# jacarvalho/mpd-public

Measured on AMD Instinct MI355X. Metric: denoising-steps/s, higher is better.
Workload: dtype f32; 1 GPU; cfg2: EnvDense2D-RobotPointMass shape, 100 trajectories (1 context(s)) x H=64 x D=4, T=100 (+5) reverse steps, unguided, U-Net dim_mults (1, 2, 4, 8), one plan = one bench step; parallelism=single, denoising_steps_per_plan=105

## Files before the change

### include/mpdx.h

```cpp
#ifndef MPDX_H
#define MPDX_H

#include <stddef.h>
#include <stdint.h>

#ifdef __cplusplus
extern "C" {
#endif

#define MPDX_E_INVALID   (-1)
#define MPDX_E_NOTFOUND  (-2)
#define MPDX_E_STATE     (-3)
#define MPDX_E_DEVICE    (-4)

#define MPDX_MAX_LEVELS 8

typedef struct mpdx_unet mpdx_unet;

typedef struct mpdx_unet_cfg {
    int32_t state_dim;
    int32_t n_support_points;
    int32_t unet_input_dim;
    int32_t n_levels;
    int32_t dim_mults[MPDX_MAX_LEVELS];
    int32_t time_emb_dim;
    int32_t self_attention;
} mpdx_unet_cfg;

const char* mpdx_last_error(void);
int mpdx_version(void);

int    mpdx_unet_create(const mpdx_unet_cfg* cfg, mpdx_unet** out);
void   mpdx_unet_destroy(mpdx_unet* u);
int    mpdx_unet_set_plan_join(mpdx_unet* u, int on);
int    mpdx_unet_plan_joined(const mpdx_unet* u);
int    mpdx_unet_set_inner_run(mpdx_unet* u, int on);
int    mpdx_unet_set_inner_run_parts(mpdx_unet* u, int parts);
int    mpdx_unet_inner_runs(const mpdx_unet* u);
int    mpdx_unet_inner_run_layers(const mpdx_unet* u);
int    mpdx_unet_status(const mpdx_unet* u);
int    mpdx_unet_set_status(mpdx_unet* u, unsigned word);
int    mpdx_unet_num_params(const mpdx_unet* u);
int    mpdx_unet_param_info(const mpdx_unet* u, int idx, const char** name, int32_t shape[3], int32_t* ndim);
size_t mpdx_unet_packed_floats(const mpdx_unet* u);
size_t mpdx_unet_timetab_floats(const mpdx_unet* u, int T);
size_t mpdx_unet_workspace_floats(const mpdx_unet* u, int B);
int    mpdx_unet_pack_param(mpdx_unet* u, const char* name, const float* src_dev, size_t n_floats,
                            float* packed_dev, void* stream);
int    mpdx_unet_build_timetab(mpdx_unet* u, const float* packed_dev, const float* freqs16_dev, int T,
                               float* timetab_dev, void* stream);

int mpdx_unet_forward(mpdx_unet* u, const float* packed_dev, const float* timetab_dev, int T,
                      const float* x, int t, float* eps, int B, float* ws, void* stream);

typedef struct mpdx_step_coefs {
    float sqrt_recip_alphas_cumprod;
    float sqrt_recipm1_alphas_cumprod;
    float posterior_mean_coef1;
    float posterior_mean_coef2;
    float noise_scale;
// ... 214 lines not shown
```

### mpd_public_amd/_lib.py

```python
from __future__ import annotations

import ctypes as C
from pathlib import Path

import os as _os

_LIB_PATH = Path(_os.environ["MPDX_LIB"]) if _os.environ.get("MPDX_LIB") else Path(__file__).resolve().parent / "libmpdx.so"
_lib = None

MAX_LEVELS = 8


class UnetCfg(C.Structure):
    _fields_ = [("state_dim", C.c_int32), ("n_support_points", C.c_int32), ("unet_input_dim", C.c_int32),
                ("n_levels", C.c_int32), ("dim_mults", C.c_int32 * MAX_LEVELS), ("time_emb_dim", C.c_int32),
                ("self_attention", C.c_int32)]


class StepCoefs(C.Structure):
    _fields_ = [("sqrt_recip_alphas_cumprod", C.c_float), ("sqrt_recipm1_alphas_cumprod", C.c_float),
                ("posterior_mean_coef1", C.c_float), ("posterior_mean_coef2", C.c_float),
                ("noise_scale", C.c_float), ("noise_std_extra", C.c_float),
                ("predict_epsilon", C.c_int32), ("clip_denoised", C.c_int32), ("ddim_k1", C.c_float), ("ddim_k2", C.c_float),
                ("guide_scale", C.c_float)]
# ... 38 lines not shown


class RrtOpts(C.Structure):
    _fields_ = [("q_lo", C.c_float * 8), ("q_hi", C.c_float * 8), ("step", C.c_float), ("max_nodes", C.c_int32), ("max_iters", C.c_int32),
                ("max_connect_steps", C.c_int32), ("n_edge_checks", C.c_int32), ("seed", C.c_uint64)]


class IkOpts(C.Structure):
    _fields_ = [("frame", C.c_int32), ("offset", C.c_float * 3), ("q_lo", C.c_float * 8), ("q_hi", C.c_float * 8), ("rot_weight", C.c_float),
                ("pos_tol", C.c_float), ("rot_tol", C.c_float), ("lambda_init", C.c_float), ("lambda_up", C.c_float), ("lambda_down", C.c_float),
                ("lambda_min", C.c_float), ("lambda_max", C.c_float), ("adaptive", C.c_int32), ("max_iters", C.c_int32), ("seed", C.c_uint64)]


_vp, _sz, _i, _f = C.c_void_p, C.c_size_t, C.c_int, C.c_float
SIGNATURES = {
    "mpdx_last_error": (C.c_char_p, []),
    "mpdx_version": (_i, []),
    "mpdx_unet_create": (_i, [C.POINTER(UnetCfg), C.POINTER(_vp)]),
    "mpdx_unet_destroy": (None, [_vp]),
    "mpdx_unet_set_plan_join": (_i, [_vp, _i]),
    "mpdx_unet_plan_joined": (_i, [_vp]),
    "mpdx_unet_set_inner_run": (_i, [_vp, _i]),
    "mpdx_unet_set_inner_run_parts": (_i, [_vp, _i]),
    "mpdx_unet_inner_runs": (_i, [_vp]),
    "mpdx_unet_inner_run_layers": (_i, [_vp]),
    "mpdx_unet_status": (_i, [_vp]),
    "mpdx_unet_set_status": (_i, [_vp, C.c_uint]),
    "mpdx_unet_num_params": (_i, [_vp]),
    "mpdx_unet_param_info": (_i, [_vp, _i, C.POINTER(C.c_char_p), C.POINTER(C.c_int32 * 3), C.POINTER(C.c_int32)]),
    "mpdx_unet_packed_floats": (_sz, [_vp]),
    "mpdx_unet_timetab_floats": (_sz, [_vp, _i]),
    "mpdx_unet_workspace_floats": (_sz, [_vp, _i]),
    "mpdx_unet_pack_param": (_i, [_vp, C.c_char_p, _vp, _sz, _vp, _vp]),
    "mpdx_unet_build_timetab": (_i, [_vp, _vp, _vp, _i, _vp, _vp]),
    "mpdx_unet_forward": (_i, [_vp, _vp, _vp, _i, _vp, _i, _vp, _i, _vp, _vp]),
    "mpdx_ddpm_step": (_i, [_vp, _vp, _vp, _i, _vp, _vp, _vp, _vp, C.POINTER(StepCoefs), _i, _i, _vp, _vp, _i, _i, _vp, _vp]),
    "mpdx_add_noise": (_i, [_vp, _vp, _vp, _vp, _f, _f, _vp, _i, _i, _i, _vp]),
    "mpdx_hard_conds": (_i, [_vp, _vp, _i, C.POINTER(C.c_int32), C.POINTER(_vp), _i, _i, _i, _vp]),
    "mpdx_q_sample": (_i, [_vp, _vp, _vp, _vp, _vp, _vp, _vp, _vp, _i, _i, _i, _i, _vp]),
    "mpdx_weighted_loss": (_i, [_vp, _vp, _vp, _vp, _vp, _i, _vp, _i, _i, _i, _vp]),
    "mpdx_plan": (_i, [_vp, _vp, _vp, _i, C.POINTER(StepCoefs), _i, _vp, _vp, _vp, _vp, _vp, _i, _vp,
                        C.POINTER(GuideParams), _i, _i, _vp, _i, C.c_uint64, C.c_uint64, _vp]),
    "mpdx_guide_step": (_i, [C.POINTER(GuideParams), _vp, _vp, _vp, _vp, _vp, _vp, _i, _i, _i, _i, _vp]),
    "mpdx_guide_step_scaled": (_i, [C.POINTER(GuideParams), _vp, _vp, _vp, _vp, _vp, _vp, _i, _i, _i, _i, _f, _vp]),
    "mpdx_guide_time": (_i, [C.POINTER(GuideParams), _vp, _vp, _vp, _i, _i, _i, _i, _i, _vp, C.POINTER(C.c_float)]),
    "mpdx_traj_metrics": (_i, [C.POINTER(GuideParams), _vp, _vp, _i, _i, _i, _i, _vp]),
# ... 85 lines not shown
```

### mpd_public_amd/csrc/host.hpp

```cpp
#pragma once
#include <hip/hip_runtime.h>

#include <algorithm>
#include <cmath>
#include <cstdarg>
#include <cstdio>
#include <cstdlib>
#include <cstring>
#include <mutex>
#include <set>
#include <string>
#include <unordered_map>
#include <vector>

#include "../../include/mpdx.h"
#include "conv_block.hpp"
#include "conv_ws.hpp"
#include "fused_level.hpp"
#include "switches.hpp"
#include "train_types.hpp"

namespace mpdx {

int fail(int code, const char* fmt, ...);
// ... 55 lines not shown
    bool pin_nt = false;
    std::string name;
};

}

struct mpdx_unet {
    mpdx_unet_cfg cfg;
    std::vector<mpdx::Param> params;
    std::unordered_map<std::string, int> pidx;
    std::vector<mpdx::Layer> layers;
    size_t packed_floats = 0;
    size_t slot_floats = 0;
    int n_slots = 0;
    int tt_row = 0;
    std::vector<int> tt_w, tt_b, tt_cout, tt_off;
    int final_slot = 0;
    int n_done = 0;
    int Hc = 0, xpad_slot = -1;
    bool masked() const { return Hc != cfg.n_support_points; }
    int plan_join = 1;
    enum RunPart { kRunSeven = 1, kRunTail = 2 };
    int inner_run = kRunSeven | kRunTail;
    int plan_joined = 0, inner_runs = 0;
    int inner_run_layers = 0;
    struct InnerRunState {
        int capacity = -1;
        bool seven_ok = false, tail_ok = false;
        long long budget = 0;
        unsigned* counters = nullptr;
        unsigned base = 0;
        int live = 1 << 30;
        bool rezero = false;
        unsigned *status = nullptr, *status_dev = nullptr;
        unsigned status_host = 0;
        unsigned status_word() const { return status ? __atomic_load_n(status, __ATOMIC_RELAXED) : status_host; }
    } run;
    struct CopyJob { size_t src, dst; int n0, ss0, ds0, n1, ss1, ds1, n_inner; };
    struct Fused {
        int first = 0, count = 0;
        bool has_final = false;
        int in1 = 0, in2 = 0;
        int in3 = mpdx::SRC_NONE;
        int gout_slot[3] = {-1, -1, -1};
        size_t lds_bytes = 0;
        mpdx::FusedArgs tmpl;
        int program = -1;
        std::vector<CopyJob> jobs;
        std::vector<int> op_layer;
        int in3_consumer = -1;
    };
    std::vector<Fused> fused;
    void* jobs_dev = nullptr;
    int n_jobs = 0;
    const float* streams_for = nullptr;
    int pack_version = 0, streams_version = -1;
    enum UnitKind { kProgram, kLayer, kPair, kInnerRun, kTailRun };
    struct Unit { UnitKind kind; int fused; int layer; int count; };
    std::vector<int> owner;
    struct TrainLayer {
        int src1_l = -2, src2_l = -2, res_l = -2;
        bool need_dgrad = false;
        size_t dgrad_woff = 0;
        mpdx::Layer dg;
    };
    bool train_ready = false;
    size_t flat_floats = 0, packedT_floats = 0;
    std::vector<TrainLayer> tl;
    std::vector<mpdx::PackDesc> pack_descs_host;
    void* pack_descs_dev = nullptr;
    void* pack_chunks_dev = nullptr;
    size_t n_pack_chunks = 0;
};

namespace mpdx {

int pick_row_stride(int cin_pad, int mode, int L_in, int L_out, int LP);
void choose_tile(const Layer& l, int B, int& MT, int& NT);
bool layer_ksplit(const Layer& l);
int check_ready(const mpdx_unet* u);
unsigned fused_mask(int B);
bool fused_save_variant(const mpdx_unet::Fused& f);
int ensure_fused_streams(mpdx_unet* u, const float* packed, hipStream_t st);
int claim_fused_stream_jobs(mpdx_unet* u, const float* packed, const void** jobs, int* n);
int launch_final_step(const FinalArgs& fa, hipStream_t st);
int launch_conv_layer(const Layer& l, ConvArgs& a, int B, hipStream_t st);
bool pair_tile(const Layer& l1, const Layer& l2, int B, int& MT, int& NT);
int launch_conv_pair(int MT, int NT, const ConvArgs& a1, const ConvArgs& a2, const Layer& l1, const Layer& l2, hipStream_t st);
template <int N> struct RunArgs;
int inner_run_grid(int B);
int inner_run_workgroups_per_cu();
int tail_run_workgroups_per_cu();
int launch_inner_run(const RunArgs<7>& ra, int B, hipStream_t st);
int launch_tail_run(const RunArgs<4>& ra, int B, hipStream_t st);
struct AttnArgs;
const char* attn_unsupported(int C, int L);
int launch_attention(const Layer& l, AttnArgs& a, int B, hipStream_t st);
int launch_weight_stationary(int variant, const Layer& l, ConvArgs& a, const ConvArgs& a2, int B, hipStream_t st);
int launch_fused_args(const mpdx_unet::Fused& f, const FusedArgs& a, int B, hipStream_t st, bool save = false);
int launch_fused_train(const mpdx_unet::Fused& f, const FusedArgs& a, int B, hipStream_t st);
int launch_fused_join(const FusedJoinArgs& ja, int B, hipStream_t st);
size_t fused_join_lds_bytes();
struct NoiseRng;
int launch_guide(const mpdx_guide_params* gp, float* x, float* grad_out, const float* hs, const float* hg, const uint32_t* amax_in,
                 uint32_t* amax_out, int n_per_ctx, int B, int H, int D, hipStream_t st, const float* noise = nullptr, float noise_scale = 0.f,
                 float noise_extra = 0.f, float* chain = nullptr, float guide_scale = 1.0f, const NoiseRng* rng = nullptr);
const char* chain_params_problem(const mpdx_guide_params& gp);
const char* tool_params_problem(const mpdx_guide_params& gp);
struct ChainInfo;
int guide_block_problem(const mpdx_guide_params* gp, int D, ChainInfo* chain_info);

}
```

### mpd_public_amd/csrc/inner_run.hpp

```cpp
#pragma once
#include "conv_block.hpp"

namespace mpdx {

constexpr int kInnerRunLayers = 7;
constexpr int kTailRunLayers = 4;
constexpr int kInnerRunCounterStride = 32;

template <int N>
struct RunArgs {
    ConvArgs layer[N];
    unsigned* counters;
    unsigned* status;
    long long budget;
    unsigned base;
    int n_layers;
    int nc;
};
typedef RunArgs<kInnerRunLayers> InnerRunArgs;
typedef RunArgs<kTailRunLayers> TailRunArgs;

constexpr size_t run_max(size_t a, size_t b) { return a > b ? a : b; }

struct RunSeqSeven {
    typedef InnerRunArgs Args;
    static constexpr int kLayers = kInnerRunLayers;
    static constexpr bool kUp = false;
    static constexpr int kLastL = 8, kLastMT = 32, kLastC = 256;
    static __device__ __forceinline__ bool gn(const ConvArgs& a, int id, const RunCtx& rc) { return conv_block_body<CONV_S1, 5, EPI_GN_MISH, 32, 32, 1, 8, GeoL8<16>, -1, true>(a, id, rc); }
    static __device__ __forceinline__ bool up(const ConvArgs&, int, const RunCtx&) { return true; }
    static __device__ __forceinline__ int tiled(int) { return 0; }
    static size_t lds() { return conv_block_lds_bytes<CONV_S1, 5, 32, 32, 8>(8, 8, 256 + 8) + 16; }
};
struct RunSeqTail {
    typedef TailRunArgs Args;
    static constexpr int kLayers = kTailRunLayers;
    static constexpr bool kUp = true;
    static constexpr int kLastL = 16, kLastMT = 16, kLastC = 128;
    static __device__ __forceinline__ bool gn(const ConvArgs& a, int id, const RunCtx& rc) { return conv_block_body<CONV_S1, 5, EPI_GN_MISH, 16, 32, 1, 8, GeoL8<8>, -1, true>(a, id, rc); }
    static __device__ __forceinline__ bool up(const ConvArgs& a, int id, const RunCtx& rc) { return conv_block_body<CONV_UPT, 4, EPI_BIAS, 16, 64, 1, 8, GeoUp8<8>, -1, true>(a, id, rc); }
    static __device__ __forceinline__ int tiled(int i) { return i >= 3 ? 1 : ((i > 0 ? 1 : 0) | (i == 2 ? 2 : 0) | 4); }
    static size_t lds() { return run_max(conv_block_lds_bytes<CONV_S1, 5, 16, 32, 8>(8, 8, 128 + 8), conv_block_lds_bytes<CONV_UPT, 4, 16, 64, 8>(8, 16, 128 + 4)) + 16; }
};

template <class SEQ>
__device__ __forceinline__ void run_give_up(const typename SEQ::Args& ra, const RunCtx& rc, const int c, const int m, const int i) {
    const int tid = threadIdx.x;
    if (tid == 0) {
        __hip_atomic_fetch_or(ra.status, 1u | ((unsigned)i << 8), __ATOMIC_RELAXED, __HIP_MEMORY_SCOPE_SYSTEM);
        __hip_atomic_store(rc.counter, rc.target + kRunPoison, __ATOMIC_RELAXED, __HIP_MEMORY_SCOPE_AGENT);
    }
    const ConvArgs& last = ra.layer[ra.n_layers - 1];
    constexpr int L = SEQ::kLastL, MT = SEQ::kLastMT;
    for (int e = tid; e < 4 * L * MT; e += 512) {
        const int b = c * 4 + (e >> geo_ilog2(L * MT)), l = (e >> geo_ilog2(MT)) & (L - 1), ch = m * MT + (e & (MT - 1));
        if (b < last.B) last.dst[((size_t)b * L + l) * SEQ::kLastC + ch] = __builtin_nanf("");
    }
}

template <class SEQ, bool SAME_XCD>
__global__ __launch_bounds__(512) void inner_run_kernel(const typename SEQ::Args ra) {
    int c, m;
    if constexpr (SAME_XCD) {
        const int b = blockIdx.x, x = b & 7, r = b >> 3;
        m = r & 7; c = (r >> 3) * 8 + x;
        if (c >= ra.nc) return;
    } else {
        c = (int)blockIdx.x >> 3; m = blockIdx.x & 7;
    }
    warm_kernarg<sizeof(typename SEQ::Args)>();
    RunCtx rc;
    rc.counter = ra.counters + (size_t)c * kInnerRunCounterStride;
    rc.budget = ra.budget;
    const int n_gn = SEQ::kUp ? ra.n_layers - 1 : ra.n_layers;
#pragma nounroll
    for (int i = 0; i < n_gn; ++i) {
        rc.wait = i > 0;
        rc.target = ra.base + 8u * (unsigned)i;
        rc.tiled = SEQ::tiled(i);
        if (SEQ::gn(ra.layer[i], c * 8 + m, rc)) continue;
        run_give_up<SEQ>(ra, rc, c, m, i);
        return;
    }
    if constexpr (SEQ::kUp) {
        rc.wait = n_gn > 0;
        rc.target = ra.base + 8u * (unsigned)n_gn;
        rc.tiled = SEQ::tiled(n_gn);
        if (!SEQ::up(ra.layer[n_gn], c * 8 + m, rc)) run_give_up<SEQ>(ra, rc, c, m, n_gn);
    }
}

// ... 2 lines not shown
```

### mpd_public_amd/csrc/k_inner_run.hip

```cpp
#include "host.hpp"
#include "inner_run.hpp"

namespace mpdx {

#ifndef MPDX_INNER_RUN_SAME_XCD
#define MPDX_INNER_RUN_SAME_XCD 1
#endif
static constexpr bool kSameXcd = MPDX_INNER_RUN_SAME_XCD != 0;

int inner_run_grid(int B) {
    const int nc = (B + 3) / 4;
    return kSameXcd ? ((nc + 7) / 8) * 64 : nc * 8;
}

template <class SEQ>
static int workgroups_per_cu() {
    int n = 0;
    if (hipOccupancyMaxActiveBlocksPerMultiprocessor(&n, (const void*)inner_run_kernel<SEQ, kSameXcd>, 512, SEQ::lds()) != hipSuccess) {
        (void)hipGetLastError();
        return 0;
    }
    return n;
}
int inner_run_workgroups_per_cu() { return workgroups_per_cu<RunSeqSeven>(); }
int tail_run_workgroups_per_cu() { return workgroups_per_cu<RunSeqTail>(); }

template <class SEQ>
static int launch_run(const typename SEQ::Args& ra, int B, hipStream_t st, const char* what) {
    if (ra.n_layers != SEQ::kLayers || ra.nc != (B + 3) / 4) return fail(MPDX_E_INVALID, "%s: %d layers, %d clusters for B=%d", what, ra.n_layers, ra.nc, B);
    hipLaunchKernelGGL((inner_run_kernel<SEQ, kSameXcd>), dim3(inner_run_grid(B)), dim3(512), SEQ::lds(), st, ra);
    return 0;
}
int launch_inner_run(const InnerRunArgs& ra, int B, hipStream_t st) { return launch_run<RunSeqSeven>(ra, B, st, "inner run"); }
int launch_tail_run(const TailRunArgs& ra, int B, hipStream_t st) { return launch_run<RunSeqTail>(ra, B, st, "tail run"); }

}
```

### mpd_public_amd/csrc/mpdx.hip

```cpp
#include "host.hpp"
#include "attn.hpp"
#include "inner_run.hpp"
#include "loss.hpp"
#include "scene_table.hpp"

namespace mpdx {

static thread_local char g_err[512] = "";
int fail(int code, const char* fmt, ...) {
    va_list ap;
    va_start(ap, fmt);
    vsnprintf(g_err, sizeof(g_err), fmt, ap);
    va_end(ap);
    return code;
}

int raise_lds_limit(const void* kern) {
    static std::mutex mu;
    static std::set<std::pair<int, const void*>> done;
    int dev = 0;
    HIP_TRY(hipGetDevice(&dev));
    std::lock_guard<std::mutex> lock(mu);
    if (done.count({dev, kern})) return 0;
    HIP_TRY(hipFuncSetAttribute(kern, hipFuncAttributeMaxDynamicSharedMemorySize, 160 * 1024));
// ... 676 lines not shown
}
static int run_fused(mpdx_unet* u, const mpdx_unet::Fused& f, const float* packed, const float* tt_row, const float* x, float* ws,
                     int B, const FinalArgs* fa, hipStream_t st) {
    if (int rc = ensure_fused_streams(u, packed, st)) return rc;
    FusedArgs a;
    if (int rc = fill_fused_args(u, f, packed, tt_row, x, ws, B, fa, a)) return rc;
    return launch_fused_args(f, a, B, st);
}
static int run_fused_join(mpdx_unet* u, const mpdx_unet::Fused& up, const mpdx_unet::Fused& dn, const float* packed, const float* tt_row, const float* tt_next,
                          const float* x, float* ws, int B, const FinalArgs* fa, hipStream_t st, long long* trace = nullptr) {
    if (int rc = ensure_fused_streams(u, packed, st)) return rc;
    FusedJoinArgs ja;
    FusedArgs d;
    if (int rc = fill_fused_args(u, up, packed, tt_row, x, ws, B, fa, ja.up)) return rc;
    if (int rc = fill_fused_args(u, dn, packed, tt_next, x, ws, B, nullptr, d)) return rc;
    ja.up.trace = trace;
    ja.dn.packed = d.packed; ja.dn.tt_row = d.tt_row;
    for (int k = 0; k < 3; ++k) ja.dn.gout[k] = d.gout[k];
    ja.dn.gpar_off = d.gpar_off; ja.dn.tt_lo = d.tt_lo;
    for (int k = 0; k < kMaxFusedOps; ++k) ja.dn.sbase[k] = k < d.nops ? d.ops[k].sbase : 0;
    return launch_fused_join(ja, B, st);
}

static size_t inner_run_counter_bytes(int capacity) { return (size_t)((capacity + 7) / 8 + 8) * kInnerRunCounterStride * sizeof(unsigned); }
static int inner_run_create(mpdx_unet::InnerRunState& r, int cus) {
    if (r.capacity >= 0) return 0;
    r.capacity = 0;
    int dev = 0, khz = 0;
    if (cus <= 0 || hipGetDevice(&dev) != hipSuccess || hipDeviceGetAttribute(&khz, hipDeviceAttributeClockRate, dev) != hipSuccess)
        return (void)hipGetLastError(), 0;
    r.seven_ok = inner_run_workgroups_per_cu() > 0;
    r.tail_ok = tail_run_workgroups_per_cu() > 0;
    if (!r.seven_ok && !r.tail_ok) return 0;
    HIP_TRY(hipMalloc((void**)&r.counters, inner_run_counter_bytes(cus)));
    HIP_TRY(hipMemset(r.counters, 0, inner_run_counter_bytes(cus)));
    HIP_TRY(hipHostMalloc((void**)&r.status, 64, hipHostMallocMapped));
    *r.status = r.status_host;
    HIP_TRY(hipHostGetDevicePointer((void**)&r.status_dev, r.status, 0));
    r.budget = 4LL * (khz > 0 ? khz : 2400000);
    r.capacity = cus;
    return 0;
}
static int inner_run_begin(mpdx_unet::InnerRunState& r, int nc, int n_layers, hipStream_t st, unsigned* base_out) {
    if (r.rezero || nc > r.live) {
        HIP_TRY(hipMemsetAsync(r.counters, 0, inner_run_counter_bytes(r.capacity), st));
        r.base = 0; r.rezero = false;
    }
    r.live = nc;
    *base_out = r.base;
    r.base += 8u * (unsigned)n_layers;
    return 0;
}
static void inner_run_free(mpdx_unet::InnerRunState& r) {
    if (r.counters) (void)hipFree(r.counters);
    if (r.status) (void)hipHostFree(r.status);
}
static int handle_status_error(const mpdx_unet* u, const char* fn) {
    const unsigned w = u->run.status_word();
    if (!w) return 0;
    return fail(MPDX_E_DEVICE, "%s: a workgroup of the inner-level run gave up its wait (status 0x%x: layer %u of the run); the outputs of that plan hold NaN. "
                "mpdx_unet_set_status(u, 0) clears the word", fn, w, w >> 8);
}
static long long* g_run_trace = nullptr;
static int g_run_trace_kind = -1;
constexpr int kRunTraceSlots = 32;
template <int N>
static int fill_run_args(mpdx_unet* u, int kind, int first, const float* packed, const float* row, const float* x, float* ws, int B, hipStream_t st, RunArgs<N>& ra) {
    memset(&ra, 0, sizeof(ra));
    for (int k = 0; k < N; ++k) {
        if (int rc = make_conv_args(u, u->layers[first + k], packed, row, x, ws, B, 0, ra.layer[k])) return rc;
        ra.layer[k].n_tiles_n = (B + 3) / 4;
        ra.layer[k].trace = g_run_trace && g_run_trace_kind == kind ? g_run_trace + k * kRunTraceSlots : nullptr;
    }
    ra.n_layers = N; ra.nc = (B + 3) / 4;
    if (int rc = inner_run_begin(u->run, ra.nc, N, st, &ra.base)) return rc;
    ra.counters = u->run.counters; ra.status = u->run.status_dev; ra.budget = u->run.budget;
    u->inner_run_layers += N;
    return 0;
}
static int run_inner_run(mpdx_unet* u, int first, const float* packed, const float* row, const float* x, float* ws, int B, hipStream_t st) {
    InnerRunArgs ra;
    if (int rc = fill_run_args(u, mpdx_unet::kInnerRun, first, packed, row, x, ws, B, st, ra)) return rc;
    u->inner_runs++;
    return launch_inner_run(ra, B, st);
}
static int run_tail_run(mpdx_unet* u, int first, int spare, const float* packed, const float* row, const float* x, float* ws, int B, hipStream_t st) {
    TailRunArgs ra;
    if (spare < 0 || spare >= u->n_slots) return fail(MPDX_E_STATE, "tail run without a spare slot");
    if (int rc = fill_run_args(u, mpdx_unet::kTailRun, first, packed, row, x, ws, B, st, ra)) return rc;
    float* const sp = ws + u->slot_floats * (size_t)B * spare;
    ra.layer[0].dst = sp; ra.layer[1].src1 = sp; ra.layer[2].res = sp;
    return launch_tail_run(ra, B, st);
}

static int run_unit(mpdx_unet* u, const mpdx_unet::Unit& un, const float* packed, const float* row, const float* x, float* ws, int B,
                    const FinalArgs* fa, hipStream_t st) {
    if (un.kind == mpdx_unet::kProgram) return run_fused(u, u->fused[un.fused], packed, row, x, ws, B, fa, st);
    if (un.kind == mpdx_unet::kPair) return run_pair(u, u->layers[un.layer], u->layers[un.layer + 1], packed, row, x, ws, B, st);
    if (un.kind == mpdx_unet::kInnerRun) return run_inner_run(u, un.layer, packed, row, x, ws, B, st);
    if (un.kind == mpdx_unet::kTailRun) return run_tail_run(u, un.layer, un.fused, packed, row, x, ws, B, st);
    return run_layer(u, u->layers[un.layer], packed, row, x, ws, B, st);
}
static double unit_flops(const mpdx_unet* u, const mpdx_unet::Unit& un, int B) {
    double fl = 0.0;
    for (int k = un.layer; k < un.layer + un.count; ++k) fl += layer_flops(u->layers[k], B);
    return fl;
}

static double layer_param_bytes(const mpdx_unet* u, const Layer& l) {
    if (l.attn) return 4.0 * ((double)u->params[l.w].n + (double)u->params[l.w2].n + 3.0 * l.cout);
    double n = (double)u->params[l.w].n + l.cout;
    if (l.gamma >= 0) n += 2.0 * l.cout;
    if (l.tb_off >= 0) n += l.cout;
    return 4.0 * n;
}
static double unit_bytes(const mpdx_unet* u, const mpdx_unet::Unit& un, int B) {
    auto act = [&](int L, int C) { return 4.0 * B * (double)L * C; };
    if (un.kind == mpdx_unet::kProgram) {
        const auto& f = u->fused[un.fused];
        const Layer& l0 = u->layers[f.first];
        double b = act(l0.L_in, l0.c1 + l0.c2);
        if (f.in3_consumer >= 0) b += act(u->layers[f.in3_consumer].L_in, u->layers[f.in3_consumer].c2);
        for (int k = f.first; k < f.first + f.count; ++k) b += layer_param_bytes(u, u->layers[k]);
// ... 111 lines not shown
        }
        if (read_later || held(u->final_slot)) continue;
        auto named = [&](const Layer& l, int s) { return l.src1 == s || l.src2 == s || l.res == s || l.dst == s; };
        for (int s = 0; s < u->n_slots && *spare < 0; ++s) {
            if (s == u->xpad_slot || named(l0, s) || named(l1, s) || named(l2, s) || named(l3, s)) continue;
            bool dead = s != u->final_slot;
            for (int j = f + kTailRunLayers; j < (int)u->layers.size() && dead; ++j) {
                const Layer& l = u->layers[j];
                if (l.src1 == s || l.src2 == s || l.res == s) dead = false;
                else if (l.dst == s) break;
            }
            if (dead) *spare = s;
        }
        if (*spare < 0 || l3.dst == l1.dst || l3.dst == l2.dst || l3.dst == l0.src1 || l3.dst == l0.res) { *spare = -1; continue; }
        return i;
    }
    return -1;
}
static int device_cus() {
    int dev = 0, cus = 0;
    if (hipGetDevice(&dev) != hipSuccess || hipDeviceGetAttribute(&cus, hipDeviceAttributeMultiprocessorCount, dev) != hipSuccess) (void)hipGetLastError();
    return cus;
}
struct PlanSchedule {
    std::vector<mpdx_unet::Unit> units;
    bool run = false;
    bool join = false;
    int build(mpdx_unet* u, int B, bool with_run = true) {
        units = current_units(u, B, nullptr);
        const int cus = device_cus();
        if (with_run && u->inner_run && !u->masked() && !u->cfg.self_attention && u->cfg.n_levels == 4 && u->cfg.n_support_points == 64) {
            if (int rc = inner_run_create(u->run, cus)) return rc;
            const bool fits = u->run.capacity > 0 && inner_run_grid(B) <= u->run.capacity && sw::geo() && !sw::debug();
            const int rf = fits && u->run.seven_ok && (u->inner_run & mpdx_unet::kRunSeven) ? inner_run_first(u, units) : -1;
            if (rf >= 0) {
                units[rf] = {mpdx_unet::kInnerRun, -1, units[rf].layer, kInnerRunLayers};
                units.erase(units.begin() + rf + 1, units.begin() + rf + kInnerRunLayers);
                run = true;
            }
            int spare = -1;
            const int tf = fits && u->run.tail_ok && (u->inner_run & mpdx_unet::kRunTail) ? tail_run_first(u, units, &spare) : -1;
            if (tf >= 0) {
                units[tf] = {mpdx_unet::kTailRun, spare, units[tf].layer, kTailRunLayers};
                units.erase(units.begin() + tf + 1, units.begin() + tf + kTailRunLayers);
                run = true;
            }
        }
        if (!u->plan_join || u->masked() || units.size() < 2) return 0;
        const mpdx_unet::Unit &first = units.front(), &last = units.back();
        if (first.kind != mpdx_unet::kProgram || last.kind != mpdx_unet::kProgram || first.fused == last.fused) return 0;
        const mpdx_unet::Fused &dn = u->fused[first.fused], &up = u->fused[last.fused];
        join = dn.program == 5 && dn.in1 == SRC_X && dn.in2 == SRC_NONE && !dn.has_final && up.program == 3 && up.has_final && B <= cus;
        return 0;
    }
};

int dev_hooks_missing(const char* fn) {
#ifdef MPDX_DEV_HOOKS
    return (void)fn, 0;
#endif
    return fail(MPDX_E_STATE, "%s needs a development build of libmpdx.so (MPDX_BUILD_DEFS=-DMPDX_DEV_HOOKS MPDX_BUILD_OUT=build_ab/libmpdx_dev.so python -m mpd_public_amd.build, then MPDX_LIB=build_ab/libmpdx_dev.so): "
                "the production kernels carry no trace / ablation hooks", fn);
}

}

// ... 45 lines not shown
    u->packed_floats += 64;
    *out = u;
    return 0;
}

int mpdx_unet_set_plan_join(mpdx_unet* u, int on) {
    if (!u) return fail(MPDX_E_INVALID, "null argument");
    u->plan_join = on ? 1 : 0;
    return 0;
}
int mpdx_unet_plan_joined(const mpdx_unet* u) { return u ? u->plan_joined : 0; }

int mpdx_unet_set_inner_run(mpdx_unet* u, int on) {
    if (!u) return fail(MPDX_E_INVALID, "null argument");
    u->inner_run = on ? (mpdx_unet::kRunSeven | mpdx_unet::kRunTail) : 0;
    return 0;
}
int mpdx_unet_set_inner_run_parts(mpdx_unet* u, int parts) {
    if (!u) return fail(MPDX_E_INVALID, "null argument");
    if (parts & ~(mpdx_unet::kRunSeven | mpdx_unet::kRunTail)) return fail(MPDX_E_INVALID, "inner-run parts 0x%x: bit 0 the seven 256 -> 256 layers, bit 1 the tail of up level 0", parts);
    u->inner_run = parts;
    return 0;
}
int mpdx_unet_inner_runs(const mpdx_unet* u) { return u ? u->inner_runs : 0; }
int mpdx_unet_inner_run_layers(const mpdx_unet* u) { return u ? u->inner_run_layers : 0; }
int mpdx_unet_status(const mpdx_unet* u) {
    if (!u) return fail(MPDX_E_INVALID, "null argument");
    return handle_status_error(u, "mpdx_unet_status");
}
int mpdx_unet_set_status(mpdx_unet* u, unsigned word) {
    if (!u) return fail(MPDX_E_INVALID, "null argument");
    if (u->run.status) __atomic_store_n(u->run.status, word, __ATOMIC_RELAXED);
    u->run.status_host = word;
    if (!word && u->run.counters) u->run.rezero = true;
    return 0;
}

void mpdx_unet_destroy(mpdx_unet* u) {
    if (u && u->pack_descs_dev) (void)hipFree(u->pack_descs_dev);
    if (u && u->pack_chunks_dev) (void)hipFree(u->pack_chunks_dev);
    if (u && u->jobs_dev) (void)hipFree(u->jobs_dev);
    if (u) inner_run_free(u->run);
    delete u;
}

int mpdx_unet_num_params(const mpdx_unet* u) { return u ? (int)u->params.size() : 0; }

int mpdx_unet_param_info(const mpdx_unet* u, int idx, const char** name, int32_t shape[3], int32_t* ndim) {
    if (!u || idx < 0 || idx >= (int)u->params.size()) return fail(MPDX_E_INVALID, "bad parameter index %d", idx);
    const Param& p = u->params[idx];
    if (name) *name = p.name.c_str();
    if (shape) { shape[0] = p.shape[0]; shape[1] = p.shape[1]; shape[2] = p.shape[2]; }
    if (ndim) *ndim = p.ndim;
    return 0;
}

size_t mpdx_unet_packed_floats(const mpdx_unet* u) { return u ? u->packed_floats : 0; }
// ... 254 lines not shown
```

### mpd_public_amd/temporal_unet.py

```python
from __future__ import annotations

import ctypes as C
import math

import torch
import torch.nn as nn

from . import _lib

UNET_DIM_MULTS = {0: (1, 2, 4), 1: (1, 2, 4, 8)}


def group_norm_n_groups(n_channels, target_n_groups=8):
    if n_channels < target_n_groups:
        return 1
    for n_groups in range(target_n_groups, target_n_groups + 10):
        if n_channels % n_groups == 0:
            return n_groups
    return 1


class _Holder(nn.Module):

    def forward(self, *a, **k):
# ... 120 lines not shown
        if self._h is None:
            lib = _lib.load()
            mults = (C.c_int32 * _lib.MAX_LEVELS)(*self.dim_mults)
            cfg = _lib.UnetCfg(int(self.state_dim), int(self.n_support_points), int(self.unet_input_dim), len(self.dim_mults),
                               mults, int(self.time_emb_dim), int(self.self_attention))
            h = C.c_void_p()
            _lib.check(lib.mpdx_unet_create(C.byref(cfg), C.byref(h)), "mpdx_unet_create")
            self._h = h
        return self._h

    def set_plan_join(self, on: bool):
        _lib.check(_lib.load().mpdx_unet_set_plan_join(self._handle(), int(bool(on))), "mpdx_unet_set_plan_join")

    def plan_joined(self) -> int:
        return int(_lib.load().mpdx_unet_plan_joined(self._handle()))

    def set_inner_run(self, on: bool):
        _lib.check(_lib.load().mpdx_unet_set_inner_run(self._handle(), int(bool(on))), "mpdx_unet_set_inner_run")

    RUN_SEVEN, RUN_TAIL = 1, 2

    def set_inner_run_parts(self, parts: int):
        _lib.check(_lib.load().mpdx_unet_set_inner_run_parts(self._handle(), int(parts)), "mpdx_unet_set_inner_run_parts")

    def inner_runs(self) -> int:
        return int(_lib.load().mpdx_unet_inner_runs(self._handle()))

    def inner_run_layers(self) -> int:
        return int(_lib.load().mpdx_unet_inner_run_layers(self._handle()))

    def status(self) -> int:
        return int(_lib.load().mpdx_unet_status(self._handle()))

    def _param_stamp(self):
        d = self.__dict__
        n = d.get("_stamp_calls", 0) + 1
        d["_stamp_calls"] = n
        pl = d.get("_plist")
        if pl is None or n % 16 == 0:
            pl = d["_plist"] = list(self.parameters())
        return tuple((p.data_ptr(), p._version) for p in pl)

    def _apply(self, fn, *a, **k):
        self.__dict__["_plist"] = None
        return super()._apply(fn, *a, **k)

# ... 70 lines not shown
```

Baseline: 6402 denoising-steps/s.

## Add narrow 16-position cluster width for persistent inner and tail runs

Parameterises the persistent inner-run and tail-run kernels on cluster width (positions per cluster). A narrower width of 16 uses half the batch rows per cluster, so the grid doubles to spread work over more CUs, with up to two resident workgroups per CU. The inner run defaults to narrow and the tail run picks narrow for B<=64 (here B=100, so wide), with separate counter regions per width. The cost is smaller N tiles and more inter-workgroup synchronisation traffic per layer.

```diff
diff --git a/include/mpdx.h b/include/mpdx.h
--- a/include/mpdx.h
+++ b/include/mpdx.h
@@ -36,6 +36,8 @@
 int    mpdx_unet_plan_joined(const mpdx_unet* u);
 int    mpdx_unet_set_inner_run(mpdx_unet* u, int on);
 int    mpdx_unet_set_inner_run_parts(mpdx_unet* u, int parts);
+int    mpdx_unet_set_inner_run_width(mpdx_unet* u, int width);
+int    mpdx_inner_run_block(int B, int width, int cus, int block, int32_t* cluster, int32_t* tile, int32_t* counter_lines);
 int    mpdx_unet_inner_runs(const mpdx_unet* u);
 int    mpdx_unet_inner_run_layers(const mpdx_unet* u);
 int    mpdx_unet_status(const mpdx_unet* u);
diff --git a/mpd_public_amd/_lib.py b/mpd_public_amd/_lib.py
--- a/mpd_public_amd/_lib.py
+++ b/mpd_public_amd/_lib.py
@@ -84,6 +84,8 @@
     "mpdx_unet_plan_joined": (_i, [_vp]),
     "mpdx_unet_set_inner_run": (_i, [_vp, _i]),
     "mpdx_unet_set_inner_run_parts": (_i, [_vp, _i]),
+    "mpdx_unet_set_inner_run_width": (_i, [_vp, _i]),
+    "mpdx_inner_run_block": (_i, [_i, _i, _i, _i, _vp, _vp, _vp]),
     "mpdx_unet_inner_runs": (_i, [_vp]),
     "mpdx_unet_inner_run_layers": (_i, [_vp]),
     "mpdx_unet_status": (_i, [_vp]),
diff --git a/mpd_public_amd/csrc/host.hpp b/mpd_public_amd/csrc/host.hpp
--- a/mpd_public_amd/csrc/host.hpp
+++ b/mpd_public_amd/csrc/host.hpp
@@ -101,16 +101,20 @@
     int plan_join = 1;
     enum RunPart { kRunSeven = 1, kRunTail = 2 };
     int inner_run = kRunSeven | kRunTail;
+    int inner_run_width = 0;
     int plan_joined = 0, inner_runs = 0;
     int inner_run_layers = 0;
     struct InnerRunState {
         int capacity = -1;
-        bool seven_ok = false, tail_ok = false;
+        int seven_wgs[2] = {0, 0}, tail_wgs[2] = {0, 0};
         long long budget = 0;
         unsigned* counters = nullptr;
-        unsigned base = 0;
-        int live = 1 << 30;
-        bool rezero = false;
+        struct Counters {
+            unsigned* p = nullptr;
+            unsigned base = 0;
+            int live = 1 << 30;
+            bool rezero = false;
+        } ctr[2];
         unsigned *status = nullptr, *status_dev = nullptr;
         unsigned status_host = 0;
         unsigned status_word() const { return status ? __atomic_load_n(status, __ATOMIC_RELAXED) : status_host; }
@@ -135,7 +139,7 @@
     const float* streams_for = nullptr;
     int pack_version = 0, streams_version = -1;
     enum UnitKind { kProgram, kLayer, kPair, kInnerRun, kTailRun };
-    struct Unit { UnitKind kind; int fused; int layer; int count; };
+    struct Unit { UnitKind kind; int fused; int layer; int count; int width = 0; };
     std::vector<int> owner;
     struct TrainLayer {
         int src1_l = -2, src2_l = -2, res_l = -2;
@@ -167,11 +171,14 @@
 bool pair_tile(const Layer& l1, const Layer& l2, int B, int& MT, int& NT);
 int launch_conv_pair(int MT, int NT, const ConvArgs& a1, const ConvArgs& a2, const Layer& l1, const Layer& l2, hipStream_t st);
 template <int N> struct RunArgs;
-int inner_run_grid(int B);
-int inner_run_workgroups_per_cu();
-int tail_run_workgroups_per_cu();
-int launch_inner_run(const RunArgs<7>& ra, int B, hipStream_t st);
-int launch_tail_run(const RunArgs<4>& ra, int B, hipStream_t st);
+bool inner_run_width_ok(int width);
+int inner_run_clusters(int B, int width);
+int inner_run_grid(int B, int width);
+void inner_run_slot(int block, int* cluster, int* tile);
+int inner_run_workgroups_per_cu(int width);
+int tail_run_workgroups_per_cu(int width);
+int launch_inner_run(const RunArgs<7>& ra, int B, int width, hipStream_t st);
+int launch_tail_run(const RunArgs<4>& ra, int B, int width, hipStream_t st);
 struct AttnArgs;
 const char* attn_unsupported(int C, int L);
 int launch_attention(const Layer& l, AttnArgs& a, int B, hipStream_t st);
diff --git a/mpd_public_amd/csrc/inner_run.hpp b/mpd_public_amd/csrc/inner_run.hpp
--- a/mpd_public_amd/csrc/inner_run.hpp
+++ b/mpd_public_amd/csrc/inner_run.hpp
@@ -6,6 +6,31 @@
 constexpr int kInnerRunLayers = 7;
 constexpr int kTailRunLayers = 4;
 constexpr int kInnerRunCounterStride = 32;
+constexpr int kRunWide = 32, kRunNarrow = 16;
+
+struct RunSlot { int c, m; };
+constexpr int run_clusters(int B, int width) { return (B + width / 8 - 1) / (width / 8); }
+constexpr int run_grid(int nc, bool same_xcd) { return same_xcd ? ((nc + 7) / 8) * 64 : nc * 8; }
+constexpr int run_block(int c, int m, bool same_xcd) { return same_xcd ? (c & 7) + 8 * (m + 8 * (c >> 3)) : 8 * c + m; }
+__host__ __device__ constexpr RunSlot run_slot(int block, bool same_xcd) {
+    return same_xcd ? RunSlot{((block >> 6) << 3) + (block & 7), (block >> 3) & 7} : RunSlot{block >> 3, block & 7};
+}
+constexpr bool run_map_ok(int width) {
+    for (int B = 1; B <= 128; ++B) {
+        const int nc = run_clusters(B, width), grid = run_grid(nc, true);
+        int live = 0;
+        for (int b = 0; b < grid; ++b) {
+            const RunSlot s = run_slot(b, true);
+            if (s.m < 0 || s.m > 7 || s.c < 0) return false;
+            if (s.c >= nc) continue;
+            if (run_block(s.c, s.m, true) != b || (b & 7) != (s.c & 7)) return false;
+            ++live;
+        }
+        if (live != 8 * nc || grid % 64 || grid < 8 * nc) return false;
+    }
+    return true;
+}
+static_assert(run_map_ok(kRunWide) && run_map_ok(kRunNarrow), "block <-> (cluster, channel tile): a bijection on the live blocks, one XCD per cluster");
 
 template <int N>
 struct RunArgs {
@@ -22,25 +47,29 @@
 
 constexpr size_t run_max(size_t a, size_t b) { return a > b ? a : b; }
 
+template <int NT>
 struct RunSeqSeven {
     typedef InnerRunArgs Args;
+    static constexpr int kWidth = NT, kSpt = NT / 8;
     static constexpr int kLayers = kInnerRunLayers;
     static constexpr bool kUp = false;
     static constexpr int kLastL = 8, kLastMT = 32, kLastC = 256;
-    static __device__ __forceinline__ bool gn(const ConvArgs& a, int id, const RunCtx& rc) { return conv_block_body<CONV_S1, 5, EPI_GN_MISH, 32, 32, 1, 8, GeoL8<16>, -1, true>(a, id, rc); }
+    static __device__ __forceinline__ bool gn(const ConvArgs& a, int id, const RunCtx& rc) { return conv_block_body<CONV_S1, 5, EPI_GN_MISH, 32, NT, 1, 8, GeoL8<16>, -1, true>(a, id, rc); }
     static __device__ __forceinline__ bool up(const ConvArgs&, int, const RunCtx&) { return true; }
     static __device__ __forceinline__ int tiled(int) { return 0; }
-    static size_t lds() { return conv_block_lds_bytes<CONV_S1, 5, 32, 32, 8>(8, 8, 256 + 8) + 16; }
+    static size_t lds() { return conv_block_lds_bytes<CONV_S1, 5, 32, NT, 8>(8, 8, 256 + 8) + 16; }
 };
+template <int NT>
 struct RunSeqTail {
     typedef TailRunArgs Args;
+    static constexpr int kWidth = NT, kSpt = NT / 8;
     static constexpr int kLayers = kTailRunLayers;
     static constexpr bool kUp = true;
     static constexpr int kLastL = 16, kLastMT = 16, kLastC = 128;
-    static __device__ __forceinline__ bool gn(const ConvArgs& a, int id, const RunCtx& rc) { return conv_block_body<CONV_S1, 5, EPI_GN_MISH, 16, 32, 1, 8, GeoL8<8>, -1, true>(a, id, rc); }
-    static __device__ __forceinline__ bool up(const ConvArgs& a, int id, const RunCtx& rc) { return conv_block_body<CONV_UPT, 4, EPI_BIAS, 16, 64, 1, 8, GeoUp8<8>, -1, true>(a, id, rc); }
+    static __device__ __forceinline__ bool gn(const ConvArgs& a, int id, const RunCtx& rc) { return conv_block_body<CONV_S1, 5, EPI_GN_MISH, 16, NT, 1, 8, GeoL8<8>, -1, true>(a, id, rc); }
+    static __device__ __forceinline__ bool up(const ConvArgs& a, int id, const RunCtx& rc) { return conv_block_body<CONV_UPT, 4, EPI_BIAS, 16, 2 * NT, 1, 8, GeoUp8<8>, -1, true>(a, id, rc); }
     static __device__ __forceinline__ int tiled(int i) { return i >= 3 ? 1 : ((i > 0 ? 1 : 0) | (i == 2 ? 2 : 0) | 4); }
-    static size_t lds() { return run_max(conv_block_lds_bytes<CONV_S1, 5, 16, 32, 8>(8, 8, 128 + 8), conv_block_lds_bytes<CONV_UPT, 4, 16, 64, 8>(8, 16, 128 + 4)) + 16; }
+    static size_t lds() { return run_max(conv_block_lds_bytes<CONV_S1, 5, 16, NT, 8>(8, 8, 128 + 8), conv_block_lds_bytes<CONV_UPT, 4, 16, 2 * NT, 8>(8, 16, 128 + 4)) + 16; }
 };
 
 template <class SEQ>
@@ -52,21 +81,18 @@
     }
     const ConvArgs& last = ra.layer[ra.n_layers - 1];
     constexpr int L = SEQ::kLastL, MT = SEQ::kLastMT;
-    for (int e = tid; e < 4 * L * MT; e += 512) {
-        const int b = c * 4 + (e >> geo_ilog2(L * MT)), l = (e >> geo_ilog2(MT)) & (L - 1), ch = m * MT + (e & (MT - 1));
+    for (int e = tid; e < SEQ::kSpt * L * MT; e += 512) {
+        const int b = c * SEQ::kSpt + (e >> geo_ilog2(L * MT)), l = (e >> geo_ilog2(MT)) & (L - 1), ch = m * MT + (e & (MT - 1));
         if (b < last.B) last.dst[((size_t)b * L + l) * SEQ::kLastC + ch] = __builtin_nanf("");
     }
 }
 
 template <class SEQ, bool SAME_XCD>
 __global__ __launch_bounds__(512) void inner_run_kernel(const typename SEQ::Args ra) {
-    int c, m;
+    const RunSlot slot = run_slot((int)blockIdx.x, SAME_XCD);
+    const int c = slot.c, m = slot.m;
     if constexpr (SAME_XCD) {
-        const int b = blockIdx.x, x = b & 7, r = b >> 3;
-        m = r & 7; c = (r >> 3) * 8 + x;
         if (c >= ra.nc) return;
-    } else {
-        c = (int)blockIdx.x >> 3; m = blockIdx.x & 7;
     }
     warm_kernarg<sizeof(typename SEQ::Args)>();
     RunCtx rc;
diff --git a/mpd_public_amd/csrc/k_inner_run.hip b/mpd_public_amd/csrc/k_inner_run.hip
--- a/mpd_public_amd/csrc/k_inner_run.hip
+++ b/mpd_public_amd/csrc/k_inner_run.hip
@@ -8,10 +8,10 @@
 #endif
 static constexpr bool kSameXcd = MPDX_INNER_RUN_SAME_XCD != 0;
 
-int inner_run_grid(int B) {
-    const int nc = (B + 3) / 4;
-    return kSameXcd ? ((nc + 7) / 8) * 64 : nc * 8;
-}
+bool inner_run_width_ok(int width) { return width == kRunWide || width == kRunNarrow; }
+int inner_run_clusters(int B, int width) { return inner_run_width_ok(width) ? run_clusters(B, width) : 0; }
+int inner_run_grid(int B, int width) { return run_grid(inner_run_clusters(B, width), kSameXcd); }
+void inner_run_slot(int block, int* cluster, int* tile) { const RunSlot s = run_slot(block, kSameXcd); *cluster = s.c; *tile = s.m; }
 
 template <class SEQ>
 static int workgroups_per_cu() {
@@ -22,16 +22,29 @@
     }
     return n;
 }
-int inner_run_workgroups_per_cu() { return workgroups_per_cu<RunSeqSeven>(); }
-int tail_run_workgroups_per_cu() { return workgroups_per_cu<RunSeqTail>(); }
+int inner_run_workgroups_per_cu(int width) {
+    return width == kRunWide ? workgroups_per_cu<RunSeqSeven<kRunWide>>() : width == kRunNarrow ? workgroups_per_cu<RunSeqSeven<kRunNarrow>>() : 0;
+}
+int tail_run_workgroups_per_cu(int width) {
+    return width == kRunWide ? workgroups_per_cu<RunSeqTail<kRunWide>>() : width == kRunNarrow ? workgroups_per_cu<RunSeqTail<kRunNarrow>>() : 0;
+}
 
 template <class SEQ>
 static int launch_run(const typename SEQ::Args& ra, int B, hipStream_t st, const char* what) {
-    if (ra.n_layers != SEQ::kLayers || ra.nc != (B + 3) / 4) return fail(MPDX_E_INVALID, "%s: %d layers, %d clusters for B=%d", what, ra.n_layers, ra.nc, B);
-    hipLaunchKernelGGL((inner_run_kernel<SEQ, kSameXcd>), dim3(inner_run_grid(B)), dim3(512), SEQ::lds(), st, ra);
+    if (ra.n_layers != SEQ::kLayers || ra.nc != run_clusters(B, SEQ::kWidth))
+        return fail(MPDX_E_INVALID, "%s: %d layers, %d clusters for B=%d at width %d", what, ra.n_layers, ra.nc, B, SEQ::kWidth);
+    hipLaunchKernelGGL((inner_run_kernel<SEQ, kSameXcd>), dim3(run_grid(ra.nc, kSameXcd)), dim3(512), SEQ::lds(), st, ra);
     return 0;
 }
-int launch_inner_run(const InnerRunArgs& ra, int B, hipStream_t st) { return launch_run<RunSeqSeven>(ra, B, st, "inner run"); }
-int launch_tail_run(const TailRunArgs& ra, int B, hipStream_t st) { return launch_run<RunSeqTail>(ra, B, st, "tail run"); }
+int launch_inner_run(const InnerRunArgs& ra, int B, int width, hipStream_t st) {
+    if (width == kRunNarrow) return launch_run<RunSeqSeven<kRunNarrow>>(ra, B, st, "inner run");
+    if (width == kRunWide) return launch_run<RunSeqSeven<kRunWide>>(ra, B, st, "inner run");
+    return fail(MPDX_E_INVALID, "inner run: width %d", width);
+}
+int launch_tail_run(const TailRunArgs& ra, int B, int width, hipStream_t st) {
+    if (width == kRunNarrow) return launch_run<RunSeqTail<kRunNarrow>>(ra, B, st, "tail run");
+    if (width == kRunWide) return launch_run<RunSeqTail<kRunWide>>(ra, B, st, "tail run");
+    return fail(MPDX_E_INVALID, "tail run: width %d", width);
+}
 
 }
diff --git a/mpd_public_amd/csrc/mpdx.hip b/mpd_public_amd/csrc/mpdx.hip
--- a/mpd_public_amd/csrc/mpdx.hip
+++ b/mpd_public_amd/csrc/mpdx.hip
@@ -722,18 +722,28 @@
     return launch_fused_join(ja, B, st);
 }
 
-static size_t inner_run_counter_bytes(int capacity) { return (size_t)((capacity + 7) / 8 + 8) * kInnerRunCounterStride * sizeof(unsigned); }
+static int run_index(int width) { return width == kRunNarrow ? 1 : 0; }
+static int inner_run_resident(int cus, int width, int wgs_per_cu) { return cus * std::min(width == kRunNarrow ? 2 : 1, wgs_per_cu); }
+static int inner_run_counter_lines(int cus, int width) { return inner_run_resident(cus, width, 2) / 8 + 8; }
+static size_t inner_run_counter_bytes(int cus, int width) { return (size_t)inner_run_counter_lines(cus, width) * kInnerRunCounterStride * sizeof(unsigned); }
 static int inner_run_create(mpdx_unet::InnerRunState& r, int cus) {
     if (r.capacity >= 0) return 0;
     r.capacity = 0;
     int dev = 0, khz = 0;
     if (cus <= 0 || hipGetDevice(&dev) != hipSuccess || hipDeviceGetAttribute(&khz, hipDeviceAttributeClockRate, dev) != hipSuccess)
         return (void)hipGetLastError(), 0;
-    r.seven_ok = inner_run_workgroups_per_cu() > 0;
-    r.tail_ok = tail_run_workgroups_per_cu() > 0;
-    if (!r.seven_ok && !r.tail_ok) return 0;
-    HIP_TRY(hipMalloc((void**)&r.counters, inner_run_counter_bytes(cus)));
-    HIP_TRY(hipMemset(r.counters, 0, inner_run_counter_bytes(cus)));
+    bool any = false;
+    for (int width : {kRunWide, kRunNarrow}) {
+        r.seven_wgs[run_index(width)] = inner_run_workgroups_per_cu(width);
+        r.tail_wgs[run_index(width)] = tail_run_workgroups_per_cu(width);
+        any = any || r.seven_wgs[run_index(width)] > 0 || r.tail_wgs[run_index(width)] > 0;
+    }
+    if (!any) return 0;
+    const size_t bytes = inner_run_counter_bytes(cus, kRunWide) + inner_run_counter_bytes(cus, kRunNarrow);
+    HIP_TRY(hipMalloc((void**)&r.counters, bytes));
+    HIP_TRY(hipMemset(r.counters, 0, bytes));
+    r.ctr[0].p = r.counters;
+    r.ctr[1].p = r.counters + inner_run_counter_lines(cus, kRunWide) * kInnerRunCounterStride;
     HIP_TRY(hipHostMalloc((void**)&r.status, 64, hipHostMallocMapped));
     *r.status = r.status_host;
     HIP_TRY(hipHostGetDevicePointer((void**)&r.status_dev, r.status, 0));
@@ -741,14 +751,17 @@
     r.capacity = cus;
     return 0;
 }
-static int inner_run_begin(mpdx_unet::InnerRunState& r, int nc, int n_layers, hipStream_t st, unsigned* base_out) {
-    if (r.rezero || nc > r.live) {
-        HIP_TRY(hipMemsetAsync(r.counters, 0, inner_run_counter_bytes(r.capacity), st));
-        r.base = 0; r.rezero = false;
-    }
-    r.live = nc;
-    *base_out = r.base;
-    r.base += 8u * (unsigned)n_layers;
+static int inner_run_begin(mpdx_unet::InnerRunState& r, int width, int nc, int n_layers, hipStream_t st, unsigned** counters_out, unsigned* base_out) {
+    mpdx_unet::InnerRunState::Counters& k = r.ctr[run_index(width)];
+    if (nc > inner_run_counter_lines(r.capacity, width)) return fail(MPDX_E_STATE, "run of width %d: %d clusters, %d counter lines", width, nc, inner_run_counter_lines(r.capacity, width));
+    if (k.rezero || nc > k.live) {
+        HIP_TRY(hipMemsetAsync(k.p, 0, inner_run_counter_bytes(r.capacity, width), st));
+        k.base = 0; k.rezero = false;
+    }
+    k.live = nc;
+    *counters_out = k.p;
+    *base_out = k.base;
+    k.base += 8u * (unsigned)n_layers;
     return 0;
 }
 static void inner_run_free(mpdx_unet::InnerRunState& r) {
@@ -765,40 +778,42 @@
 static int g_run_trace_kind = -1;
 constexpr int kRunTraceSlots = 32;
 template <int N>
-static int fill_run_args(mpdx_unet* u, int kind, int first, const float* packed, const float* row, const float* x, float* ws, int B, hipStream_t st, RunArgs<N>& ra) {
+static int fill_run_args(mpdx_unet* u, int kind, int first, int width, const float* packed, const float* row, const float* x, float* ws, int B, hipStream_t st, RunArgs<N>& ra) {
     memset(&ra, 0, sizeof(ra));
+    if (!inner_run_width_ok(width)) return fail(MPDX_E_STATE, "run unit of width %d", width);
+    const int nc = inner_run_clusters(B, width);
     for (int k = 0; k < N; ++k) {
         if (int rc = make_conv_args(u, u->layers[first + k], packed, row, x, ws, B, 0, ra.layer[k])) return rc;
-        ra.layer[k].n_tiles_n = (B + 3) / 4;
+        ra.layer[k].n_tiles_n = nc;
         ra.layer[k].trace = g_run_trace && g_run_trace_kind == kind ? g_run_trace + k * kRunTraceSlots : nullptr;
     }
-    ra.n_layers = N; ra.nc = (B + 3) / 4;
-    if (int rc = inner_run_begin(u->run, ra.nc, N, st, &ra.base)) return rc;
-    ra.counters = u->run.counters; ra.status = u->run.status_dev; ra.budget = u->run.budget;
+    ra.n_layers = N; ra.nc = nc;
+    if (int rc = inner_run_begin(u->run, width, nc, N, st, &ra.counters, &ra.base)) return rc;
+    ra.status = u->run.status_dev; ra.budget = u->run.budget;
     u->inner_run_layers += N;
     return 0;
 }
-static int run_inner_run(mpdx_unet* u, int first, const float* packed, const float* row, const float* x, float* ws, int B, hipStream_t st) {
+static int run_inner_run(mpdx_unet* u, int first, int width, const float* packed, const float* row, const float* x, float* ws, int B, hipStream_t st) {
     InnerRunArgs ra;
-    if (int rc = fill_run_args(u, mpdx_unet::kInnerRun, first, packed, row, x, ws, B, st, ra)) return rc;
+    if (int rc = fill_run_args(u, mpdx_unet::kInnerRun, first, width, packed, row, x, ws, B, st, ra)) return rc;
     u->inner_runs++;
-    return launch_inner_run(ra, B, st);
-}
-static int run_tail_run(mpdx_unet* u, int first, int spare, const float* packed, const float* row, const float* x, float* ws, int B, hipStream_t st) {
+    return launch_inner_run(ra, B, width, st);
+}
+static int run_tail_run(mpdx_unet* u, int first, int spare, int width, const float* packed, const float* row, const float* x, float* ws, int B, hipStream_t st) {
     TailRunArgs ra;
     if (spare < 0 || spare >= u->n_slots) return fail(MPDX_E_STATE, "tail run without a spare slot");
-    if (int rc = fill_run_args(u, mpdx_unet::kTailRun, first, packed, row, x, ws, B, st, ra)) return rc;
+    if (int rc = fill_run_args(u, mpdx_unet::kTailRun, first, width, packed, row, x, ws, B, st, ra)) return rc;
     float* const sp = ws + u->slot_floats * (size_t)B * spare;
     ra.layer[0].dst = sp; ra.layer[1].src1 = sp; ra.layer[2].res = sp;
-    return launch_tail_run(ra, B, st);
+    return launch_tail_run(ra, B, width, st);
 }
 
 static int run_unit(mpdx_unet* u, const mpdx_unet::Unit& un, const float* packed, const float* row, const float* x, float* ws, int B,
                     const FinalArgs* fa, hipStream_t st) {
     if (un.kind == mpdx_unet::kProgram) return run_fused(u, u->fused[un.fused], packed, row, x, ws, B, fa, st);
     if (un.kind == mpdx_unet::kPair) return run_pair(u, u->layers[un.layer], u->layers[un.layer + 1], packed, row, x, ws, B, st);
-    if (un.kind == mpdx_unet::kInnerRun) return run_inner_run(u, un.layer, packed, row, x, ws, B, st);
-    if (un.kind == mpdx_unet::kTailRun) return run_tail_run(u, un.layer, un.fused, packed, row, x, ws, B, st);
+    if (un.kind == mpdx_unet::kInnerRun) return run_inner_run(u, un.layer, un.width, packed, row, x, ws, B, st);
+    if (un.kind == mpdx_unet::kTailRun) return run_tail_run(u, un.layer, un.fused, un.width, packed, row, x, ws, B, st);
     return run_layer(u, u->layers[un.layer], packed, row, x, ws, B, st);
 }
 static double unit_flops(const mpdx_unet* u, const mpdx_unet::Unit& un, int B) {
@@ -956,6 +971,8 @@
     if (hipGetDevice(&dev) != hipSuccess || hipDeviceGetAttribute(&cus, hipDeviceAttributeMultiprocessorCount, dev) != hipSuccess) (void)hipGetLastError();
     return cus;
 }
+static int inner_run_auto_width(int B) { return (void)B, kRunNarrow; }
+static int tail_run_auto_width(int B) { return B <= 64 ? kRunNarrow : kRunWide; }
 struct PlanSchedule {
     std::vector<mpdx_unet::Unit> units;
     bool run = false;
@@ -965,17 +982,23 @@
         const int cus = device_cus();
         if (with_run && u->inner_run && !u->masked() && !u->cfg.self_attention && u->cfg.n_levels == 4 && u->cfg.n_support_points == 64) {
             if (int rc = inner_run_create(u->run, cus)) return rc;
-            const bool fits = u->run.capacity > 0 && inner_run_grid(B) <= u->run.capacity && sw::geo() && !sw::debug();
-            const int rf = fits && u->run.seven_ok && (u->inner_run & mpdx_unet::kRunSeven) ? inner_run_first(u, units) : -1;
+            const bool may = u->run.capacity > 0 && sw::geo() && !sw::debug();
+            auto width_of = [&](const int (&wgs)[2], int automatic) {
+                auto fits = [&](int w) { return may && inner_run_grid(B, w) <= inner_run_resident(u->run.capacity, w, wgs[run_index(w)]); };
+                if (u->inner_run_width) return fits(u->inner_run_width) ? u->inner_run_width : 0;
+                return fits(automatic) ? automatic : fits(kRunWide) ? kRunWide : 0;
+            };
+            const int sw7 = width_of(u->run.seven_wgs, inner_run_auto_width(B)), swt = width_of(u->run.tail_wgs, tail_run_auto_width(B));
+            const int rf = sw7 && (u->inner_run & mpdx_unet::kRunSeven) ? inner_run_first(u, units) : -1;
             if (rf >= 0) {
-                units[rf] = {mpdx_unet::kInnerRun, -1, units[rf].layer, kInnerRunLayers};
+                units[rf] = {mpdx_unet::kInnerRun, -1, units[rf].layer, kInnerRunLayers, sw7};
                 units.erase(units.begin() + rf + 1, units.begin() + rf + kInnerRunLayers);
                 run = true;
             }
             int spare = -1;
-            const int tf = fits && u->run.tail_ok && (u->inner_run & mpdx_unet::kRunTail) ? tail_run_first(u, units, &spare) : -1;
+            const int tf = swt && (u->inner_run & mpdx_unet::kRunTail) ? tail_run_first(u, units, &spare) : -1;
             if (tf >= 0) {
-                units[tf] = {mpdx_unet::kTailRun, spare, units[tf].layer, kTailRunLayers};
+                units[tf] = {mpdx_unet::kTailRun, spare, units[tf].layer, kTailRunLayers, swt};
                 units.erase(units.begin() + tf + 1, units.begin() + tf + kTailRunLayers);
                 run = true;
             }
@@ -1067,6 +1090,23 @@
     u->inner_run = parts;
     return 0;
 }
+int mpdx_unet_set_inner_run_width(mpdx_unet* u, int width) {
+    if (!u) return fail(MPDX_E_INVALID, "null argument");
+    if (width != 0 && !inner_run_width_ok(width)) return fail(MPDX_E_INVALID, "inner-run width %d: 0 (automatic), 16 or 32 positions per cluster", width);
+    u->inner_run_width = width;
+    return 0;
+}
+int mpdx_inner_run_block(int B, int width, int cus, int block, int32_t* cluster, int32_t* tile, int32_t* counter_lines) {
+    if (B <= 0 || cus <= 0 || !inner_run_width_ok(width)) return fail(MPDX_E_INVALID, "mpdx_inner_run_block: B=%d width=%d cus=%d", B, width, cus);
+    const int grid = inner_run_grid(B, width);
+    if (block < 0 || block >= grid) return fail(MPDX_E_INVALID, "mpdx_inner_run_block: block %d of %d", block, grid);
+    int c = 0, m = 0;
+    inner_run_slot(block, &c, &m);
+    if (cluster) *cluster = c < inner_run_clusters(B, width) ? c : -1;
+    if (tile) *tile = m;
+    if (counter_lines) *counter_lines = inner_run_counter_lines(cus, width);
+    return grid;
+}
 int mpdx_unet_inner_runs(const mpdx_unet* u) { return u ? u->inner_runs : 0; }
 int mpdx_unet_inner_run_layers(const mpdx_unet* u) { return u ? u->inner_run_layers : 0; }
 int mpdx_unet_status(const mpdx_unet* u) {
@@ -1077,7 +1117,7 @@
     if (!u) return fail(MPDX_E_INVALID, "null argument");
     if (u->run.status) __atomic_store_n(u->run.status, word, __ATOMIC_RELAXED);
     u->run.status_host = word;
-    if (!word && u->run.counters) u->run.rezero = true;
+    if (!word && u->run.counters) u->run.ctr[0].rezero = u->run.ctr[1].rezero = true;
     return 0;
 }
 
diff --git a/mpd_public_amd/temporal_unet.py b/mpd_public_amd/temporal_unet.py
--- a/mpd_public_amd/temporal_unet.py
+++ b/mpd_public_amd/temporal_unet.py
@@ -166,6 +166,9 @@
 
     def set_inner_run_parts(self, parts: int):
         _lib.check(_lib.load().mpdx_unet_set_inner_run_parts(self._handle(), int(parts)), "mpdx_unet_set_inner_run_parts")
+
+    def set_inner_run_width(self, width: int):
+        _lib.check(_lib.load().mpdx_unet_set_inner_run_width(self._handle(), int(width)), "mpdx_unet_set_inner_run_width")
 
     def inner_runs(self) -> int:
         return int(_lib.load().mpdx_unet_inner_runs(self._handle()))
```

After: 6469 denoising-steps/s, median of 6. 1.01x the previous value.
